# leggedrobotics/open3d_slam_private

Measured on AMD Instinct MI355X. Metric: ICP iterations/sec (scan-to-map), higher is better.
Workload: dtype f32

## Files before the change

open3d_slam_private_amd/capi.py:

```python
from __future__ import annotations

import ctypes as C
import math
import os
import subprocess

import numpy as np

_HERE = os.path.dirname(os.path.abspath(__file__))
_SO = os.environ.get("O3D_REG_LIB") or os.path.join(_HERE, "lib", "libo3dslam_reg.so")

STATUS_NAMES = {0: "OK", 1: "EMPTY_TARGET", 2: "EMPTY_SOURCE", 3: "NO_CORRESPONDENCES", 4: "BAD_TRANSFORM",
                5: "NOT_CONFIGURED", 6: "BAD_ARGUMENT", 7: "MISSING_FIELD", 8: "DEVICE_ERROR", 9: "UNSUPPORTED",
                10: "OUT_OF_BOUNDS"}
OUT_OF_BOUNDS = 10
COST_P2PL, COST_GICP = 0, 1
COST_O3D_P2PL, COST_O3D_P2P = 2, 3
SMOOTH_LEN_MAX = 15


class RegError(RuntimeError):
    def __init__(self, status, msg=""):
        self.status = status
        super().__init__(f"{STATUS_NAMES.get(status, status)}: {msg}")
# ... 1528 lines not shown
        raise RegError(st, "reg_host_o3d_update")
    return U.reshape(4, 4).T.copy(), rank.value


def host_tail_plan(n, cus=256, tile=0):
    lib = load_library()
    lib.reg_host_tail_plan.argtypes = [C.c_int64, C.c_int32, C.c_int32, C.POINTER(C.c_int32)]
    lib.reg_host_tail_plan.restype = None
    out = (C.c_int32 * 4)()
    lib.reg_host_tail_plan(int(n), int(cus), int(tile), out)
    return bool(out[0]), int(out[1]), int(out[2]), int(out[3])


def host_predict_band(limit, prev=math.inf, prev2=math.inf, last_count=0, last_lo=math.inf, last_hi=math.inf, debug_narrow=0):
    lib = load_library()
    lib.reg_host_predict_band.argtypes = [C.c_float, C.c_float, C.c_float, C.c_uint32, C.c_float, C.c_float, C.c_int32,
                                          C.POINTER(C.c_float), C.POINTER(C.c_float)]
    lib.reg_host_predict_band.restype = None
    out = (C.c_float * 2)()
    lib.reg_host_predict_band(float(limit), float(prev), float(prev2), int(last_count), float(last_lo), float(last_hi),
                              int(debug_narrow), out, None)
    return np.float32(out[0]), np.float32(out[1])


def host_band_constants():
    lib = load_library()
    lib.reg_host_predict_band.argtypes = [C.c_float, C.c_float, C.c_float, C.c_uint32, C.c_float, C.c_float, C.c_int32,
                                          C.POINTER(C.c_float), C.POINTER(C.c_float)]
    lib.reg_host_predict_band.restype = None
    c = (C.c_float * 8)()
    lib.reg_host_predict_band(math.inf, math.inf, math.inf, 0, math.inf, math.inf, 0, None, c)
    names = ("band_cap", "wide_rel", "floor", "ratio_max", "centre_gain", "geom_rel", "guard_frac", "forced_wide")
    return {k: float(np.float32(v)) for k, v in zip(names, c)}
```

open3d_slam_private_amd/csrc/host_loop.hpp:

```cpp
#pragma once


static reg_status check_ready(reg_handle* h, bool need_prepared) {
    if (!h) return REG_BAD_ARGUMENT;
    if (!h->device_ok) return REG_DEVICE_ERROR;
    if (h->m == 0) {
        h->err = "no reference set (reg_set_target)";
        return REG_NOT_CONFIGURED;
    }
    if (h->n == 0) {
        h->err = "no reading set (reg_set_source)";
        return REG_NOT_CONFIGURED;
    }
    if (need_prepared && !h->prepared) {
        h->err = "reg_prepare has not been called for this reading";
        return REG_NOT_CONFIGURED;
    }
    return REG_OK;
}

static reg_status prepare_rowmajor(reg_handle* h, const float* T_init_row, const float* c_override = nullptr,
                                   int64_t n_global = 0, const IterState* init_state = nullptr) {
    reg_status s = check_ready(h, false);
    if (s != REG_OK) return s;
// ... 278 lines not shown
    const float* B = m->T_prev;
    float R[9];
    for (int i = 0; i < 3; ++i)
        for (int j = 0; j < 3; ++j) R[3 * i + j] = A[4 * i + 0] * B[4 * j + 0] + A[4 * i + 1] * B[4 * j + 1] + A[4 * i + 2] * B[4 * j + 2];
    float t[3];
    for (int i = 0; i < 3; ++i) t[i] = A[4 * i + 3] - (R[3 * i + 0] * B[3] + R[3 * i + 1] * B[7] + R[3 * i + 2] * B[11]);
    *trans = std::sqrt(t[0] * t[0] + t[1] * t[1] + t[2] * t[2]);
    const float sx = 0.5f * (R[7] - R[5]), sy = 0.5f * (R[2] - R[6]), sz = 0.5f * (R[3] - R[1]);
    *rot = std::sqrt(sx * sx + sy * sy + sz * sz);
}

static reg_status enqueue_tail(reg_handle* h, const TailPlan& pl, int max_iters) {
    if (!h->i_tail_sync.p) h->tail_sync_dirty = true;
    HIPCHK(h, h->i_tail_sync.reserve(2 * (size_t)kTailSyncBytes));
    if (h->tail_sync_dirty) {
        HIPCHK(h, hipMemsetAsync(h->i_tail_sync.p, 0, 2 * (size_t)kTailSyncBytes, h->stream));
        h->tail_sync_dirty = false;
    }
    const int sync_slot = h->tail_sync_slot;
    h->tail_sync_slot ^= 1;
    h->tail_sync_last = sync_slot;
    unsigned* const sync_cur = h->i_tail_sync.as<unsigned>() + (size_t)sync_slot * (kTailSyncBytes / 4);
    unsigned* const sync_next = h->i_tail_sync.as<unsigned>() + (size_t)(sync_slot ^ 1) * (kTailSyncBytes / 4);
    HIPCHK(h, h->i_tail_rows.reserve((size_t)2 * pl.grid * kTailHistRow * 8));
    HIPCHK(h, h->i_tail_band.reserve((size_t)2 * kTailBandCap * kTailRec * 4));
    const FilterCfg f = make_filter_cfg(h, 0);
    TailCfg cfg;
    cfg.n = h->n;
    cfg.chunk8 = pl.chunk8;
    cfg.wpc = pl.wpc;
    cfg.tile = pl.tile;
    cfg.max_iters = std::max(1, std::min(max_iters, kTailMaxIters));
    cfg.slack = coherent_slack(h);
    cfg.seq = ++h->seq;
    cfg.timeout_ticks = (unsigned long long)(h->env.tail_timeout_s * 1e8);
    uint8_t* hint = h->dbg.match_variant == 2 ? nullptr : h->i_hint.as<uint8_t>();
    const bool gicp = h->prm.cost == REG_COST_GICP;
    const float4* s_attr = gicp ? (const float4*)h->s_cov.as<float4>() : (const float4*)(h->has_snrm ? h->s_nrm.as<float4>() : nullptr);
    const float4* t_attr = gicp ? (const float4*)h->t_cov.as<float4>() : (const float4*)h->t_nrm.as<float4>();
    auto go = [&](auto kernel) {
        launch_timed(h, 3, kernel, dim3(pl.grid), dim3(kTailThreads), kTailLdsBytes, (const float4*)h->s_xyz.as<float4>(), s_attr,
                     h->i_iter.as<IterState>(), h->grid, t_attr, f, h->i_pos.as<int>(), h->i_d2.as<float>(), h->i_w.as<float>(), hint,
                     h->i_cache.as<float4>(), sync_cur, h->i_tail_rows.as<double>(), h->i_tail_band.as<float>(), h->d_mirror, cfg,
                     sync_next);
    };
    if (gicp)
        go(k_tail<true>);
    else
        go(k_tail<false>);
    HIPCHK(h, hipGetLastError());
    h->have_match = true;
    return REG_OK;
}

static reg_status enqueue_iteration(reg_handle* h, bool want_w) {
    reg_status s = enqueue_match(h);
    if (s != REG_OK) return s;
    if (h->prm.cost == REG_COST_P2PL && h->prm.use_trimmed) enqueue_select(h);
    return enqueue_linearize(h, want_w);
}

static inline unsigned long long mirror_seq(const reg_handle* h) {
    return __atomic_load_n(&h->h_mirror->seq, __ATOMIC_ACQUIRE);
}

static reg_status wait_seq(reg_handle* h, unsigned long long seq) {
// ... 168 lines not shown
                  std::fabs(in.limit_last - in.limit_prev) <= settle_tol * in.limit_last;
    }
    if (settled && in.any && (p.p2pl || p.fixed <= 0) && (p.can_fuse || tail_now)) {
        if (in.step_trans > p.settle_trans || in.step_rot > p.settle_rot) settled = false;
    }
    if (!(p.can_fuse || tail_now) || in.generic_left > 0 || !settled) return {SteerChoice::kGeneric, 1};
    const int rest = in.limit - (in.completed + in.inflight);
    if (tail_now) return {SteerChoice::kTail, rest};
    return {SteerChoice::kFused, p.fixed > 0 && !p.no_burst ? rest : 1};
}

static reg_status wait_tail(reg_handle* h, unsigned long long tail_seq, Lookahead& la, bool* tail_off) {
    const HostMirror* mir = h->h_mirror;
    for (unsigned spins = 0;; ++spins) {
        const unsigned long long m = mirror_seq(h);
        if (m >= tail_seq) break;
        if (m + 1 == tail_seq) {
            const HostMirror::SeqRecord* rec = &mir->ring[(tail_seq - 1) % kSeqRing];
            if (__atomic_load_n(&rec->seq, __ATOMIC_ACQUIRE) == tail_seq - 1 && (rec->done || rec->stall)) break;
        }
        __builtin_ia32_pause();
        if ((spins & 0xfff) == 0xfff) {
            const hipError_t e = hipStreamQuery(h->stream);
            if (e == hipSuccess) break;
            if (e != hipErrorNotReady) {
                h->tail_sync_dirty = true;
                h->err = std::string("device fault while waiting for the tail kernel: ") + hipGetErrorString(e);
                return REG_DEVICE_ERROR;
            }
        }
    }
    const bool reported = mirror_seq(h) >= tail_seq;
    const unsigned* sync_last = h->i_tail_sync.as<unsigned>() + (size_t)h->tail_sync_last * (kTailSyncBytes / 4);
    unsigned words[4] = {0, 0, 0, 0};
    if (!reported || h->env.coh_stats || mir->status == REG_DEVICE_ERROR)
        (void)hipMemcpy(words, sync_last + kTailErrWord, sizeof(words), hipMemcpyDeviceToHost);
    if (words[0] != 0 || (reported && mir->status == REG_DEVICE_ERROR)) {
        h->tail_sync_dirty = true;
        h->err = "persistent tail kernel: a grid barrier timed out (workgroups not co-resident? another process "
                 "running a persistent kernel on this GPU?); set O3D_NO_TAIL=1 to use the three-launch iteration";
        return REG_DEVICE_ERROR;
    }
    if (!reported && !(mir->stall && std::max(mirror_seq(h), la.seq0) > la.acked)) la.acked = h->seq;
    if (h->env.coh_stats)
        fprintf(stderr, "[o3dreg] tail launch: %u iterations, %u point searches (%.2f %% of the point-iterations), stall cause %u, band records of its last iteration %d\n", words[2],
                words[1], words[2] ? 100.0 * words[1] / ((double)words[2] * (double)h->n) : 0.0, words[3], reported ? mir->pad_nband : -1);
    if (reported) h->last_tail_iters += mir->pad3;
    if (reported && mir->stall && h->prm.fixed_iters <= 0) *tail_off = true;
#if O3D_TAIL_STAMPS
    {
        unsigned long long st[24];
        (void)hipMemcpy(st, sync_last + kTailStampWord, sizeof(st), hipMemcpyDeviceToHost);
        const double it_n = std::max(1, reported ? mir->pad3 : 1);
        static const char* names[12] = {"check", "search", "epilogue", "bandrec+comps", "sum+publish+drain", "arrive+wait", "row sums",
                                        "band-stage", "band-scan", "band-rank", "band-add", "solve+update"};
        for (int wg = 0; wg < 2; ++wg) {
            fprintf(stderr, "[o3dreg] tail stamps (us per iteration, %s workgroup):", wg ? "last" : "first");
            for (int i = 0; i < 12; ++i) fprintf(stderr, " %s %.2f", names[i], st[12 * wg + i] * 0.01 / it_n);
            fprintf(stderr, "\n");
        }
    }
#endif
    return REG_OK;
}

static reg_status loop_time_end(reg_handle* h, bool event_timing, std::chrono::steady_clock::time_point t_begin, float* loop_ms) {
    if (event_timing) {
        HIPCHK(h, hipEventRecord(h->ev1, h->stream));
        HIPCHK(h, hipEventSynchronize(h->ev1));
        (void)hipEventElapsedTime(loop_ms, h->ev0, h->ev1);
    } else {
        *loop_ms = std::chrono::duration<float, std::milli>(std::chrono::steady_clock::now() - t_begin).count();
    }
    return REG_OK;
}

static void loop_end_diagnostics(reg_handle* h, reg_result* res) {
    const HostMirror* mir = h->h_mirror;
    if (h->env.hints) {
// ... 31 lines not shown
            }
        }
        for (hipEvent_t e : h->prof_ev) (void)hipEventDestroy(e);
        h->prof_ev.clear();
        h->prof_kind.clear();
        h->profiling = false;
    }
}

static reg_status register_pm(reg_handle* h, const float* Ti, float T_out[16], reg_result* res);

extern "C" {

void reg_host_tail_plan(int64_t n, int32_t cus, int32_t tile, int32_t plan[4]) {
    const TailPlan pl = tail_plan_for(n, cus, 0, tile);
    plan[0] = pl.ok ? 1 : 0;
    plan[1] = pl.grid;
    plan[2] = pl.wpc;
    plan[3] = pl.chunk8;
}

REG_API void reg_host_predict_band(float limit, float prev, float prev2, uint32_t last_count, float last_lo, float last_hi,
                                   int32_t debug_narrow, float band[2], float consts[8]) {
    const Band b = predict_band(limit, prev, prev2, last_count, last_lo, last_hi, debug_narrow);
    if (band) {
        band[0] = b.lo;
        band[1] = b.hi;
    }
    if (consts) {
        const float c[8] = {(float)kTailBandCap, kTailWideRel, kBandFloor, kBandRatioMax, kBandCentreGain, kBandGeomRel, kBandGuardFrac,
                            kBandForcedWide};
        for (int i = 0; i < 8; ++i) consts[i] = c[i];
    }
}

reg_status reg_prepare(reg_handle* h, const float T_init[16]) {
    if (!h || !T_init) return REG_BAD_ARGUMENT;
    float Tr[16];
    col_to_row(T_init, Tr);
    return prepare_rowmajor(h, Tr);
}

reg_status reg_linearize(reg_handle* h, const float T_iter[16], float H[36], float b[6], double* err,
                         int64_t* n_inliers) {
    reg_status s = check_ready(h, true);
    if (s != REG_OK) return s;
    if (!T_iter) return REG_BAD_ARGUMENT;
    if (h->prm.cost == REG_COST_O3D_P2P) {
        h->err = "reg_linearize: point-to-point (Umeyama) has no normal equations";
        return REG_UNSUPPORTED;
    }
    if (h->pm_on) {
        h->err = "reg_linearize: not available with a libpointmatcher chain (reg_set_pm_chain)";
        return REG_UNSUPPORTED;
    }
    float Tr[16];
    col_to_row(T_iter, Tr);
    if (!m4_is_finite(Tr)) return REG_BAD_TRANSFORM;
    HIPCHK(h, hipSetDevice(h->prm.device));
    s = iterate_once(h, Tr, true);
    if (s != REG_OK) return s;
    const double* sums = h->h_mirror->sums;
    if (H && b) sums_to_system(sums, h->prm.cost, H, b);
    if (err) *err = sums[27];
    if (n_inliers) *n_inliers = (int64_t)llround(sums[28]);
    if (sums[28] == 0.0) {
// ... 221 lines not shown
```

open3d_slam_private_amd/csrc/host_target.hpp:

```cpp
#pragma once



struct DevBuf {
    void* p = nullptr;
    size_t cap = 0;
    hipError_t reserve(size_t bytes) {
        if (bytes <= cap) return hipSuccess;
        if (p) (void)hipFree(p);
        p = nullptr;
        cap = 0;
        hipError_t e = hipMalloc(&p, bytes ? bytes : 16);
        if (e == hipSuccess) cap = bytes;
        return e;
    }
    void release() {
        if (p) (void)hipFree(p);
        p = nullptr;
        cap = 0;
    }
    template <class T>
    T* as() const {
        return (T*)p;
    }
};

struct EnvSwitches {
    bool trace = false;
    bool event_timing = false;
    bool halo_occ = true;
    bool no_dynprune = false;
    bool no_empty_bound = false;
    bool no_witness = false;
    bool no_burst = false;
    bool hints = false;
    bool stamps = false;
    bool coh_stats = false;
    bool tail_always = false;
    bool update_generic = false;
    bool no_tail = false;
    int tail_wpc = 0;
    double dist_timeout_s = 30.0;
    float tail_timeout_s = 2.f;
    int xcd_tile_first = 32;
    int xcd_tile_later = 16;
    float settle_trans = 0.02f;
    float settle_rot = 4e-3f;
    int tail_min_iters = 8;
    int tail_tile = 0;
    bool no_gicp_tail = false;
    int gicp_tail_after = 1;
    float tail_settle_tol = 1.2f;
    int lookahead = 2;
    float settle_tol = 0.05f;
    float halo_ratio = 1.25f;
    float halo_rho = 0.4f;
    float reach_bins = 7.25f;
    float bin_occupancy = 8.f;
    float level_ratio = 2.0f;
    void read() {
        trace = getenv("O3D_TRACE") != nullptr;
        event_timing = getenv("O3D_EVENT_TIMING") != nullptr;
        no_burst = getenv("O3D_NO_BURST") != nullptr;
        no_dynprune = getenv("O3D_NO_DYNPRUNE") != nullptr;
        no_empty_bound = getenv("O3D_NO_EMPTY_BOUND") != nullptr;
        no_witness = getenv("O3D_NO_WITNESS") != nullptr;
        halo_occ = getenv("O3D_NO_HALO_OCC") == nullptr;
        hints = getenv("O3D_HINTS") != nullptr;
        stamps = getenv("O3D_STAMPS") != nullptr;
        coh_stats = getenv("O3D_COH_STATS") != nullptr;
        tail_always = getenv("O3D_TAIL_ALWAYS") != nullptr;
        no_tail = getenv("O3D_NO_TAIL") != nullptr;
        if (const char* v = getenv("O3D_UPDATE_GENERIC")) update_generic = atoi(v) != 0;
        if (const char* v = getenv("O3D_TAIL_WPC")) tail_wpc = std::max(0, atoi(v));
        if (const char* v = getenv("O3D_DIST_TIMEOUT_S")) dist_timeout_s = std::max(0.5, atof(v));
        if (const char* v = getenv("O3D_TAIL_SETTLE")) tail_settle_tol = (float)atof(v);
        if (const char* v = getenv("O3D_NO_GICP_TAIL")) no_gicp_tail = atoi(v) != 0;
        if (const char* v = getenv("O3D_TAIL_TILE")) tail_tile = std::max(0, atoi(v));
        if (const char* v = getenv("O3D_TAIL_MIN_ITERS")) tail_min_iters = std::max(0, atoi(v));
        if (const char* v = getenv("O3D_SETTLE_TRANS")) settle_trans = (float)atof(v);
        if (const char* v = getenv("O3D_SETTLE_ROT")) settle_rot = (float)atof(v);
        if (const char* v = getenv("O3D_XCD_TILE_FIRST")) xcd_tile_first = std::max(0, atoi(v));
        if (const char* v = getenv("O3D_XCD_TILE_LATER")) xcd_tile_later = std::max(0, atoi(v));
        if (const char* v = getenv("O3D_GICP_TAIL_AFTER")) gicp_tail_after = atoi(v);
        if (const char* v = getenv("O3D_TAIL_TIMEOUT_S")) tail_timeout_s = std::min(30.f, std::max(0.01f, (float)atof(v)));
        if (const char* v = getenv("O3D_KAHEAD")) lookahead = std::max(1, atoi(v));
        if (const char* v = getenv("O3D_SETTLE")) settle_tol = (float)atof(v);
        if (const char* v = getenv("O3D_HALO_RATIO")) halo_ratio = std::min(4.0f, std::max(0.5f, (float)atof(v)));
        if (const char* v = getenv("O3D_HALO_RHO")) halo_rho = std::min(1.0f, std::max(0.05f, (float)atof(v)));
        if (const char* v = getenv("O3D_REACH_BINS")) reach_bins = std::max(1.0f, (float)atof(v));
        if (const char* v = getenv("O3D_BIN_OCC")) bin_occupancy = std::min(64.0f, std::max(1.0f, (float)atof(v)));
        if (const char* v = getenv("O3D_LEVEL_RATIO")) level_ratio = std::min(4.0f, std::max(1.2f, (float)atof(v)));
    }
};

struct DistCtx;

struct reg_handle {
    reg_params prm;
    reg_debug_params dbg;
    EnvSwitches env;
    std::string err;
    hipStream_t stream = nullptr;
    bool own_stream = false;
    bool device_ok = false;
// ... 1299 lines not shown
```

open3d_slam_private_amd/csrc/kernels_tail.hpp:

```cpp
#pragma once

#ifndef O3D_TAIL_ACQ
#define O3D_TAIL_ACQ 0
#endif
#ifndef O3D_TAIL_THREADS
#define O3D_TAIL_THREADS 512
#endif
constexpr int kTailThreads = O3D_TAIL_THREADS;
#ifndef O3D_TAIL_SLOTS
#define O3D_TAIL_SLOTS 1024
#endif
#ifndef O3D_TAIL_WGS_PER_CU
#define O3D_TAIL_WGS_PER_CU 1
#endif
constexpr int kTailSlots = O3D_TAIL_SLOTS;
constexpr int kTailWgsPerCu = O3D_TAIL_WGS_PER_CU;
constexpr int kTailPts = kTailSlots / kTailThreads;
constexpr int kTailRec = 12;
constexpr int kTailHistRow = 32;
constexpr int kTailCoarse = 256;
constexpr int kTailMaxIters = 64;
constexpr int kTailSyncWords = 256;
constexpr int kTailRing = 4;
constexpr int kTailBandCntWord = 128;
constexpr int kTailAccRows = 16;
constexpr int kTailAccDoubles = kTailRing * kTailAccRows * kSums;
constexpr int kTailSyncBytes = kTailSyncWords * 4 + kTailAccDoubles * 8;
constexpr int kTailArriveStride = 16;
constexpr int kTailErrWord = 192;
constexpr int kTailSearchedWord = 193;
constexpr int kTailItersWord = 194;
constexpr int kTailCauseWord = 195;
constexpr int kTailStampWord = 200;
constexpr int kTailGroups = kTailThreads / 8;
constexpr int kTailBins = 1024;
#ifndef O3D_TAIL_STAMPS
#define O3D_TAIL_STAMPS 0
#endif
#ifndef O3D_TAIL_G4
#define O3D_TAIL_G4 0
#endif
#if O3D_TAIL_STAMPS
#define TAIL_STAMP(i)                                                      \
    do {                                                                   \
        const unsigned long long now_ = __builtin_amdgcn_s_memrealtime();  \
        stamp_acc[i] += now_ - stamp_last;                                 \
        stamp_last = now_;                                                 \
    } while (0)
#else
#define TAIL_STAMP(i) do { } while (0)
#endif

struct TailCfg {
    int64_t n;
    int chunk8;
    int wpc;
    int tile;
    int max_iters;
    float slack;
    unsigned long long seq;
    unsigned long long timeout_ticks;
};

struct TailLds {
    static constexpr int kRows = 0;
    static constexpr int kUnion = kRows + 5 * kTailSlots * 16;
    static constexpr int kUnionSeg = (kTailThreads / 8) * kSegWords<8> * 4, kUnionSeg4 = O3D_TAIL_G4 ? (kTailThreads / 4) * kSegWords<4> * 4 : 0;
    static constexpr int kUnionMax = kUnionSeg > kUnionSeg4 ? (kUnionSeg > kTailBandCap * 8 ? kUnionSeg : kTailBandCap * 8)
                                                            : (kUnionSeg4 > kTailBandCap * 8 ? kUnionSeg4 : kTailBandCap * 8);
    static constexpr int kUnionBytes = (kUnionMax + 255) & ~255;
    static constexpr int kD2 = kUnion + kUnionBytes;
    static constexpr int kFail = kD2 + kTailSlots * 4;
    static constexpr int kWcls = kFail + kTailSlots * 2;
    static constexpr int kHint = kWcls + kTailSlots;
    static constexpr int kSh = kHint + kTailSlots;
    static constexpr int kTot = kSh + 16 * kSums * 8;
    static constexpr int kState = kTot + kSums * 8;
    static constexpr int kStateBytes = (int)((sizeof(IterState) + 15) & ~size_t(15));
    static constexpr int kMisc = kState + kStateBytes;
    static constexpr int kWtot = kMisc + 64;
    static constexpr int kOff = kWtot + 64;
    static constexpr int kX = kOff + 272 * 4;
    static constexpr int kWork = kX + 96;
    static constexpr int kMirror = kWork + kUpdWorkBytes;
    static constexpr int kMirrorBytes = (int)((sizeof(HostMirror) + 15) & ~size_t(15));
    static constexpr int kHist = kMirror + kMirrorBytes;
    static constexpr int kTotal = kHist + kTailBins * 4;
    static constexpr int kBk = kUnion;
};
static_assert(TailLds::kBk + kTailBandCap * 8 - TailLds::kUnion <= TailLds::kUnionBytes, "phase-C scratch exceeds the union");
static_assert(kTailGroups * kSegWords<8> * 4 <= TailLds::kUnionBytes, "segment lists exceed the union");
static_assert(TailLds::kTotal * kTailWgsPerCu <= 160 * 1024, "LDS budget of one CU");
constexpr int kTailLdsBytes = TailLds::kTotal;

__device__ __forceinline__ double tail_ld_f64(const double* p) {
    const unsigned long long v = __hip_atomic_load(reinterpret_cast<unsigned long long*>(const_cast<double*>(p)), __ATOMIC_RELAXED,
                                                   __HIP_MEMORY_SCOPE_AGENT);
    return __longlong_as_double((long long)v);
}
__device__ __forceinline__ void tail_st_f64(double* p, double x) {
    __hip_atomic_store(reinterpret_cast<unsigned long long*>(p), (unsigned long long)__double_as_longlong(x), __ATOMIC_RELAXED,
                       __HIP_MEMORY_SCOPE_AGENT);
}
__device__ __forceinline__ unsigned long long tail_ld_u64(const void* p) {
    return __hip_atomic_load(reinterpret_cast<unsigned long long*>(const_cast<void*>(p)), __ATOMIC_RELAXED, __HIP_MEMORY_SCOPE_AGENT);
}
__device__ __forceinline__ void tail_st_u64(void* p, unsigned long long x) {
    __hip_atomic_store(reinterpret_cast<unsigned long long*>(p), x, __ATOMIC_RELAXED, __HIP_MEMORY_SCOPE_AGENT);
}
__device__ __forceinline__ unsigned tail_ld_u32(const unsigned* p) {
    return __hip_atomic_load(const_cast<unsigned*>(p), __ATOMIC_RELAXED, __HIP_MEMORY_SCOPE_AGENT);
}

__device__ __noinline__ __attribute__((flatten)) void tail_solve_update(IterState* sit, const double* tot, const uint32_t* misc, float* s_x, UpdWork* work,
                                               bool trim, unsigned n_band_raw, unsigned n_band_all) {
    const int lane = (int)(threadIdx.x & 63);
    const float r_limit_last = sit->limit_last, r_limit_sel = __uint_as_float(misc[2]);
    const int r_dbg_narrow = sit->debug_narrow_band & 1;
    const int r_fixed = sit->fixed_iters, r_iters = sit->iterations;
    const int r_xnc = sit->xicp_nc;
    const double r_tot28 = tot[28];
    float r_T[16];
#pragma unroll
    for (int i = 0; i < 16; ++i) r_T[i] = sit->T[i];
    const int r = lane >> 3, c = lane & 7;
    double a = 0.0;
// ... 250 lines not shown
            sit->chk.max_iter_reached = true;
            sit->done = 1;
        }
    }
}

template <bool kGicp>
__global__ void __launch_bounds__(kTailThreads, (kTailThreads / 256) * kTailWgsPerCu)
k_tail(const float4* __restrict__ src, const float4* __restrict__ src_nrm ,
       IterState* __restrict__ it_g, Grid g, const float4* __restrict__ tgt_nrm ,
       FilterCfg f, int* __restrict__ pos_io, float* __restrict__ d2_out,
       float* __restrict__ w_out, uint8_t* __restrict__ hint_g, float4* __restrict__ cache, unsigned* __restrict__ sync,
       double* __restrict__ hist_g , float* __restrict__ band_g ,
       HostMirror* host, TailCfg cfg, unsigned* __restrict__ sync_next ) {
    extern __shared__ __attribute__((aligned(16))) char lds[];
    float4* const st_rows = reinterpret_cast<float4*>(lds + TailLds::kRows);
    uint32_t* const seg_lds = reinterpret_cast<uint32_t*>(lds + TailLds::kUnion);
    unsigned long long* const bk = reinterpret_cast<unsigned long long*>(lds + TailLds::kBk);
    float* const d2s = reinterpret_cast<float*>(lds + TailLds::kD2);
    uint16_t* const fail = reinterpret_cast<uint16_t*>(lds + TailLds::kFail);
    uint8_t* const wcls = reinterpret_cast<uint8_t*>(lds + TailLds::kWcls);
    uint8_t* const hnt = reinterpret_cast<uint8_t*>(lds + TailLds::kHint);
    double (*const sh)[kSums] = reinterpret_cast<double (*)[kSums]>(lds + TailLds::kSh);
    double* const tot = reinterpret_cast<double*>(lds + TailLds::kTot);
    uint32_t* const s_state = reinterpret_cast<uint32_t*>(lds + TailLds::kState);
    IterState* const sit = reinterpret_cast<IterState*>(s_state);
    uint32_t* const misc = reinterpret_cast<uint32_t*>(lds + TailLds::kMisc);
    uint32_t* const wtot = reinterpret_cast<uint32_t*>(lds + TailLds::kWtot);
    uint32_t* const off = reinterpret_cast<uint32_t*>(lds + TailLds::kOff);
    float* const s_x = reinterpret_cast<float*>(lds + TailLds::kX);
    UpdWork* const work = reinterpret_cast<UpdWork*>(lds + TailLds::kWork);
    uint32_t* const mir_w = reinterpret_cast<uint32_t*>(lds + TailLds::kMirror);
    uint32_t* const hist = reinterpret_cast<uint32_t*>(lds + TailLds::kHist);
    double* const acc_g = reinterpret_cast<double*>(sync + kTailSyncWords);
    constexpr int kStateWords = (int)(sizeof(IterState) / 4);
    constexpr int kWaves = kTailThreads / 64;
    static_assert(kStateWords <= kTailThreads && kTailThreads >= 256, "state staging / count scan by the first threads");

    const int t = threadIdx.x, lane = t & 63, wave = t >> 6;
    const int nwg = (int)gridDim.x;
    const int xcls = (int)(blockIdx.x & 7), wq = (int)(blockIdx.x >> 3);
    const int64_t n = cfg.n;
    int64_t q[kTailPts];
    bool valid[kTailPts];
    float4 s[kTailPts], sn[kTailPts];
    float4 sc1[kTailPts];
#pragma unroll
    for (int u = 0; u < kTailPts; ++u) {
        const int sl = t + u * kTailThreads;
        const int64_t oc = (int64_t)(sl >> 3) * cfg.wpc + wq;
        const int64_t r_in = oc * 8 + (sl & 7);
        if (cfg.tile > 0) {
            const int64_t tl = oc / cfg.tile, rr = oc - tl * cfg.tile;
            q[u] = ((tl * 8 + xcls) * cfg.tile + rr) * 8 + (sl & 7);
        } else {
            q[u] = (int64_t)xcls * cfg.chunk8 + r_in;
        }
        valid[u] = r_in < cfg.chunk8 && q[u] < n;
        if (!valid[u]) q[u] = 0;
    }
    if (t < kStateWords) s_state[t] = reinterpret_cast<const uint32_t*>(it_g)[t];
#pragma unroll
    for (int u = 0; u < kTailPts; ++u) {
        const int sl = t + u * kTailThreads;
        float4 r0 = cache[q[u]], r1 = cache[(size_t)n + q[u]];
        const float4 r2 = cache[2 * (size_t)n + q[u]], r3 = cache[3 * (size_t)n + q[u]];
// ... 112 lines not shown
    auto reserve_records = [&](unsigned set, const bool (&mine)[kTailPts], unsigned (&slot)[kTailPts]) {
        unsigned long long bal[kTailPts];
        unsigned nw = 0;
#pragma unroll
        for (int u = 0; u < kTailPts; ++u) {
            bal[u] = __ballot(mine[u]);
            nw += (unsigned)__popcll(bal[u]);
        }
        unsigned base = 0;
        if (nw != 0u) {
            if (lane == 0) base = atomicAdd(&sync[kTailBandCntWord + 16 * set], nw);
            base = (unsigned)__shfl((int)base, 0);
        }
        unsigned before = 0;
#pragma unroll
        for (int u = 0; u < kTailPts; ++u) {
            slot[u] = base + before + (unsigned)__popcll(bal[u] & ((1ull << lane) - 1ull));
            before += (unsigned)__popcll(bal[u]);
        }
    };
    auto store_record = [&](int buf, unsigned slotb, const float (&F)[7], float md2, float w) {
        if (slotb >= (unsigned)kTailBandCap) return;
        float* rec = band_g + ((size_t)buf * kTailBandCap + slotb) * kTailRec;
        const float kept = w != 0.f ? 1.f : 0.f;
        const float v[12] = {F[0], F[1], F[2], F[3], F[4], F[5], F[6], md2, kept, 0.f, w != 0.f ? md2 : 0.f, 0.f};
#pragma unroll
        for (int k = 0; k < 6; ++k)
            tail_st_u64(rec + 2 * k, ((unsigned long long)__float_as_uint(v[2 * k + 1]) << 32) | __float_as_uint(v[2 * k]));
    };

    for (;; ++k_local) {
        tv = t;
        asm volatile("" : "+v"(tv));
        Xf T;
#pragma unroll
        for (int k = 0; k < 12; ++k) T.m[k] = __int_as_float(__builtin_amdgcn_readfirstlane(__float_as_int(sit->T[k])));
        const float band_lo = sit->band_lo, band_hi = sit->band_hi;
        const bool trim = !kGicp && sit->use_trim && sit->trim_ratio != 1.0f;
        const bool wide = trim && band_hi < INFINITY && (band_hi - band_lo) > kTailWideRel * band_lo;
        const uint32_t u_lo = __float_as_uint(band_lo), u_hi = __float_as_uint(band_hi);
        const double f_scale = (wide ? (double)kTailCoarse : 1.0) / (double)(u_hi > u_lo ? u_hi - u_lo : 1u);
        auto coarse_bin = [&](float d2) -> uint32_t {
            return min((uint32_t)((double)(__float_as_uint(d2) - u_lo) * f_scale), (uint32_t)(kTailCoarse - 1));
        };
        float3 p[kTailPts];
#pragma unroll
        for (int u = 0; u < kTailPts; ++u) {
            const int sl = t + u * kTailThreads;
            p[u] = xf_point(T, s[u].x, s[u].y, s[u].z);
            const float4 c = st_rows[sl], tq = st_rows[kTailSlots + sl], nn = st_rows[2 * kTailSlots + sl],
                         ru = st_rows[3 * kTailSlots + sl];
            const int pprev = __float_as_int(tq.w);
            bool pass = false;
            const float attr_ok = kGicp ? st_rows[4 * kTailSlots + sl].w : nn.w;
            if (valid[u] && c.w > 0.f && pprev >= 0 && attr_ok == 1.f) {
                const float dx = p[u].x - tq.x, dy = p[u].y - tq.y, dz = p[u].z - tq.z;
                float a = dx * dx;
                float b2 = dy * dy;
                float d2 = a + b2;
                a = dz * dz;
                d2 = d2 + a;
                const float ex = p[u].x - c.x, ey = p[u].y - c.y, ez = p[u].z - c.z;
                const float delta = __builtin_amdgcn_sqrtf(ex * ex + ey * ey + ez * ez);
                const float lhs = (__builtin_amdgcn_sqrtf(d2) + delta) * 1.00001f + 1e-30f;
                const float rhs = __builtin_amdgcn_sqrtf(c.w) * 0.99999f;
                pass = d2 <= g.max_d2 && lhs < rhs;
                if (ru.w == 1.f) {
                    const float fx = p[u].x - ru.x, fy = p[u].y - ru.y, fz = p[u].z - ru.z;
                    float a2 = fx * fx;
                    float b3 = fy * fy;
                    float r2 = a2 + b3;
                    a2 = fz * fz;
                    r2 = r2 + a2;
                    pass = pass && d2 < r2;
                }
                if (pass) d2s[sl] = d2;
            }
            if (valid[u] && !pass) {
                const unsigned at = atomicAdd(&misc[0], 1u);
                fail[at] = (uint16_t)sl;
                st_rows[sl] = make_float4(p[u].x, p[u].y, p[u].z, -1.f);
            }
        }
        __syncthreads();
        TAIL_STAMP(0);
        const int nf = (int)misc[0];
        n_searched += (t == 0) ? (unsigned)nf : 0u;
        auto search_rounds = [&](auto gtag) {
            constexpr int G = decltype(gtag)::value;
            constexpr int kGroups = kTailThreads / G;
            const int sub = t & (G - 1), grp = t / G;
            for (int base = 0; base < nf; base += kGroups) {
                const int fi = base + grp;
                if (fi < nf) {
                    const int slot = (int)fail[fi];
                    const float4 a0 = st_rows[slot];
                    const float3 p2 = make_float3(a0.x, a0.y, a0.z);
                    const int hv = (int)hnt[slot];
                    int lvl;
                    float cov2;
                    const Best bb = nearest_group<G, O3D_COH_PRUNE != 0, true>(g, p2, sub, -1, &lvl, seg_lds + grp * kSegWords<G>,
                                                                               hv >= 2 ? hv - 2 : -1, &cov2, cfg.slack);
                    if (sub == 0) {
                        hnt[slot] = (uint8_t)(lvl + 1);
                        st_rows[slot] = make_float4(p2.x, p2.y, p2.z, bb.pos >= 0 ? fminf(bb.third, cov2) : -1.f);
                        st_rows[kTailSlots + slot].w = __int_as_float(bb.pos);
                        st_rows[3 * kTailSlots + slot].w = __int_as_float(bb.pos2);
                        d2s[slot] = bb.pos >= 0 ? bb.d2 : INFINITY;
                    }
                }
            }
        };
#if O3D_TAIL_G4
        if (nf > kTailThreads / 8)
            search_rounds(std::integral_constant<int, 4>());
        else
#endif
            search_rounds(std::integral_constant<int, 8>());
        __syncthreads();
#pragma unroll 1
        for (int fi = tv; fi < nf; fi += kTailThreads) {
            const int slot = (int)fail[fi];
            const int pos = __float_as_int(st_rows[kTailSlots + slot].w), pos2 = __float_as_int(st_rows[3 * kTailSlots + slot].w);
            const size_t pc = (size_t)(pos >= 0 ? pos : 0), pc2 = (size_t)(pos2 >= 0 ? pos2 : 0);
            const float4 t2 = g.pts[pc2];
            float4 tq = kGicp ? g.pts[pc] : tgt_nrm[2 * pc];
            float4 nn = kGicp ? tgt_nrm[2 * pc] : tgt_nrm[2 * pc + 1];
            if (kGicp) {
                float4 c1 = tgt_nrm[2 * pc + 1];
                c1.w = 1.f;
                st_rows[4 * kTailSlots + slot] = c1;
            } else {
                nn.w = 1.f;
            }
            tq.w = __int_as_float(pos);
            st_rows[kTailSlots + slot] = tq;
            st_rows[2 * kTailSlots + slot] = nn;
            st_rows[3 * kTailSlots + slot] = pos2 >= 0 ? make_float4(t2.x, t2.y, t2.z, 1.f)
                                                       : make_float4(INFINITY, INFINITY, INFINITY, 1.f);
        }
        __syncthreads();
        TAIL_STAMP(1);
        float rF[kTailPts][7], md2v[kTailPts], wv[kTailPts];
        int clsv[kTailPts];
        const unsigned set = epoch & (kTailRing - 1);
        int buf = (int)(epoch & 1u);
        {
            double v[kSums];
#pragma unroll
            for (int k = 0; k < kSums; ++k) v[k] = 0.0;
#pragma unroll
            for (int u = 0; u < kTailPts; ++u) {
                const int sl = t + u * kTailThreads;
#pragma unroll
                for (int k = 0; k < 7; ++k) rF[u][k] = 0.f;
                const float4 tq = st_rows[kTailSlots + sl], nn = st_rows[2 * kTailSlots + sl];
                const int mpos = valid[u] ? __float_as_int(tq.w) : -1;
                const float md2 = d2s[sl];
                float w = 0.f;
                int cls = 2;
                if (kGicp) {
                    if (valid[u] && mpos >= 0) {
                        w = 1.f;
                        cls = 0;
                        tail_gicp_factor(T, s[u], sn[u], sc1[u], tq, nn, st_rows[4 * kTailSlots + sl], md2, v);
                    }
                } else if (valid[u] && mpos >= 0) {
                    w = 1.f;
                    if (f.use_maxdist && !(md2 <= f.outlier_max_d2)) w = 0.f;
                    if (f.use_normal) {
                        const float3 nr = normalize3(xf_rot(T, sn[u].x, sn[u].y, sn[u].z));
                        const float3 nt = normalize3(make_float3(nn.x, nn.y, nn.z));
                        float a = nr.x * nt.x;
                        float bb2 = nr.y * nt.y;
                        float val = a + bb2;
                        a = nr.z * nt.z;
                        val = val + a;
                        if (val < f.cos_max_angle) w = 0.f;
                    }
                    cls = md2 < band_lo ? 0 : (md2 < band_hi ? 1 : 2);
                    if (w != 0.f && cls != 2) {
                        float a = p[u].y * nn.z, bq = p[u].z * nn.y;
                        rF[u][0] = a - bq;
                        a = p[u].z * nn.x; bq = p[u].x * nn.z;
                        rF[u][1] = a - bq;
                        a = p[u].x * nn.y; bq = p[u].y * nn.x;
                        rF[u][2] = a - bq;
                        rF[u][3] = nn.x; rF[u][4] = nn.y; rF[u][5] = nn.z;
                        const float dx = p[u].x - tq.x, dy = p[u].y - tq.y, dz = p[u].z - tq.z;
                        float r = dx * nn.x;
                        float t2 = dy * nn.y;
                        r = r + t2;
                        t2 = dz * nn.z;
                        r = r + t2;
                        rF[u][6] = r;
                    }
                    v[29] += 1.0;
                    if (cls == 0) v[31] += 1.0;
                    if (w != 0.f && cls == 0) accumulate(v, rF[u], md2);
                }
                if (!(valid[u] && mpos >= 0)) d2s[sl] = INFINITY;
                wcls[sl] = (uint8_t)((w != 0.f && cls != 2 ? 1 : 0) | (cls << 1));
                md2v[u] = md2;
                wv[u] = w;
                clsv[u] = cls;
                if (wide && cls == 1) atomicAdd(&hist[coarse_bin(md2)], 1u);
            }
            unsigned slot[kTailPts];
            if (!wide) {
                bool mine[kTailPts];
#pragma unroll
                for (int u = 0; u < kTailPts; ++u) mine[u] = clsv[u] == 1;
                reserve_records(set, mine, slot);
            }
            publish_sums(v);
            if (!wide) {
#pragma unroll
                for (int u = 0; u < kTailPts; ++u)
                    if (clsv[u] == 1) store_record(buf, slot[u], rF[u], md2v[u], wv[u]);
            }
        }
        TAIL_STAMP(2);
        if (wide) {
            __syncthreads();
            if (t < kTailCoarse / 8) {
                unsigned long long pk = 0ull;
#pragma unroll
                for (int j = 0; j < 8; ++j) {
                    const uint32_t c2 = hist[8 * t + j];
                    hist[8 * t + j] = 0u;
                    pk |= (unsigned long long)min(c2, 255u) << (8 * j);
                }
                tail_st_u64(hist_g + ((size_t)buf * nwg + blockIdx.x) * kTailHistRow + tv, pk);
            }
        }
        if (t == 0) {
            misc[0] = 0u;
            misc[5] = 0u;
            misc[9] = 0u;
            misc[2] = __float_as_uint(INFINITY);
        }
        TAIL_STAMP(3);
        if (!exchange(set)) {
            exit_reason = 4;
            if (t == 0) __hip_atomic_fetch_add(&sync[kTailErrWord], 1u, __ATOMIC_RELAXED, __HIP_MEMORY_SCOPE_AGENT);
            break;
        }
        TAIL_STAMP(5);
        uint32_t sel_bin = 0;
        bool stall = false;
        unsigned rset = set;
        unsigned long long rv[6] = {0ull, 0ull, 0ull, 0ull, 0ull, 0ull};
        unsigned n_band_raw = 0;
        auto load_records_spec = [&]() {
            n_band_raw = tail_ld_u32(&sync[kTailBandCntWord + 16 * rset]);
            const float* rec = band_g + ((size_t)buf * kTailBandCap + (unsigned)tv) * kTailRec;
#pragma unroll
            for (int k = 0; k < 6; ++k) rv[k] = tail_ld_u64(rec + 2 * k);
        };
        if (!wide) load_records_spec();
        reduce_sums(set, false);
        TAIL_STAMP(6);
        if (trim && wide && (uint32_t)llround(tot[29]) != 0u) {
            {
                const unsigned* wbase = reinterpret_cast<const unsigned*>(hist_g + (size_t)buf * nwg * kTailHistRow) + (tv & 63);
                constexpr int kG = kTailThreads / 64, kL = (256 * kTailWgsPerCu) / kG;
                unsigned c4[4] = {0, 0, 0, 0};
                bool sat = false;
                for (int u0 = 0; u0 < kL; u0 += 8) {
                    unsigned wv2[8];
// ... 174 lines not shown
                    const float d2r = __uint_as_float((unsigned)(r6[3] >> 32)), keptr = __uint_as_float((unsigned)r6[4]);
                    if (i < n_band && d2r <= limit && keptr != 0.f) {
                        const float F[7] = {__uint_as_float((unsigned)r6[0]), __uint_as_float((unsigned)(r6[0] >> 32)),
                                            __uint_as_float((unsigned)r6[1]), __uint_as_float((unsigned)(r6[1] >> 32)),
                                            __uint_as_float((unsigned)r6[2]), __uint_as_float((unsigned)(r6[2] >> 32)),
                                            __uint_as_float((unsigned)r6[3])};
                        accumulate(v, F, d2r);
                    }
                }
                wave_reduce32(v);
                if ((lane & 1) == 0) sh[wave][lane >> 1] = v[0];
                __syncthreads();
                if (t < kSums) {
                    double v2 = 0.0;
#pragma unroll
                    for (int w2 = 0; w2 < kWaves; ++w2) v2 += sh[w2][t];
                    tot[t] += v2;
                }
                __syncthreads();
            }
        }
        TAIL_STAMP(10);
        if (t < kSums) sit->sums[t] = tot[t];
        if (wave == 0) {
            if (kGicp)
                tail_solve_update_gicp(sit, tot, reinterpret_cast<double*>(s_x), work);
            else
                tail_solve_update(sit, tot, misc, s_x, work, trim, n_band_raw, wide ? misc[12] : n_band_raw);
        }
        __syncthreads();
        TAIL_STAMP(11);
        if (sit->done) {
            exit_reason = 1;
            ++k_local;
            break;
        }
        if (k_local + 1 >= cfg.max_iters) {
            exit_reason = 3;
            ++k_local;
            break;
        }
    }
    if (exit_reason == 2 || exit_reason == 4) {
        if (t == 0) {
            sit->stall = 1;
            sit->band_count = 0;
        }
        __syncthreads();
    }
#pragma unroll
    for (int u = 0; u < kTailPts; ++u) {
        if (!valid[u]) continue;
        const int sl = t + u * kTailThreads;
        const float4 tq = st_rows[kTailSlots + sl];
        const int cls = (int)(wcls[sl] >> 1);
        float w = (wcls[sl] & 1) ? 1.f : 0.f;
        if (cls == 1 && !(d2s[sl] <= __uint_as_float(misc[2]))) w = 0.f;
        pos_io[q[u]] = __float_as_int(tq.w);
        d2_out[q[u]] = d2s[sl];
        if (w_out) w_out[q[u]] = w;
        if (hint_g) hint_g[q[u]] = hnt[sl];
    }
    if (exit_reason == 3) {
        for (int sl = t; sl < kTailSlots; sl += kTailThreads) {
            const int64_t oc = (int64_t)(sl >> 3) * cfg.wpc + wq;
            const int64_t r_in = oc * 8 + (sl & 7);
            int64_t qq;
            if (cfg.tile > 0) {
                const int64_t tl = oc / cfg.tile, rr = oc - tl * cfg.tile;
                qq = ((tl * 8 + xcls) * cfg.tile + rr) * 8 + (sl & 7);
            } else {
                qq = (int64_t)xcls * cfg.chunk8 + r_in;
            }
            if (r_in < cfg.chunk8 && qq < n) {
#pragma unroll
                for (int r = 0; r < 4; ++r) cache[(size_t)r * (size_t)n + qq] = st_rows[r * kTailSlots + sl];
            }
        }
    }
    if (t == 0 && n_searched) atomicAdd(&sync[kTailSearchedWord], n_searched);
#if O3D_TAIL_STAMPS
    if (t == 0 && (blockIdx.x == 0 || blockIdx.x == gridDim.x - 1)) {
        unsigned long long* out = reinterpret_cast<unsigned long long*>(sync + kTailStampWord) + (blockIdx.x == 0 ? 0 : 12);
        for (int i = 0; i < 12; ++i) out[i] = stamp_acc[i];
    }
#endif
    if (blockIdx.x != 0) return;
    for (int w2 = t; w2 < kTailSyncBytes / 4; w2 += kTailThreads) sync_next[w2] = 0u;
    if (t == 0) sync[kTailItersWord] = (unsigned)k_local;
    if (wave != 0) return;
    if (lane == 0) {
        HostMirror* m = reinterpret_cast<HostMirror*>(mir_w);
        for (int i = 0; i < 16; ++i) m->T[i] = sit->T[i];
        for (int i = 0; i < 16; ++i) m->T_prev[i] = sit->T_prev[i];
        m->iterations = sit->iterations;
        m->done = sit->done;
        m->status = exit_reason == 4 ? (int)REG_DEVICE_ERROR : sit->status;
        m->rank_last = sit->rank_last;
        m->converged = sit->chk.converged ? 1 : 0;
        m->max_iter_reached = sit->chk.max_iter_reached ? 1 : 0;
        m->stall = sit->stall;
        m->band_count = (int)sit->band_count;
        m->limit_last = sit->limit_last;
        m->limit_prev = sit->limit_prev;
        m->band_lo = sit->band_lo;
        m->band_hi = sit->band_hi;
        m->pad_nband = (int)sit->band_count;
        m->pad2 = exit_reason;
        for (int i = 0; i < 6; ++i) {
            m->localizable[i] = sit->xicp_flags[i];
            m->xicp_comb[i] = sit->xicp_comb[i];
            m->xicp_high[i] = sit->xicp_high[i];
        }
// ... 30 lines not shown
```

Measured before the change: 19040.

## Skip nearest-neighbour searches for points certainly trimmed in the tail kernel

In the persistent tail kernel, a point whose cached match fails the coherence check is no longer re-searched if a distance bound shows it will certainly fall above the trim band's upper edge. Such points are marked trimmed (class 2) and counted. A final verification pass runs on convergence to re-check skipped points, using the final transform kept in LDS. This cuts k-d/grid search work per iteration, at the cost of extra LDS, a possible extra pass at convergence, and more branching. An environment variable turns it off.

After: 18760. 0.985x the previous value.

```diff
diff --git a/open3d_slam_private_amd/capi.py b/open3d_slam_private_amd/capi.py
--- a/open3d_slam_private_amd/capi.py
+++ b/open3d_slam_private_amd/capi.py
@@ -1584,3 +1584,18 @@
     lib.reg_host_predict_band(math.inf, math.inf, math.inf, 0, math.inf, math.inf, 0, None, c)
     names = ("band_cap", "wide_rel", "floor", "ratio_max", "centre_gain", "geom_rel", "guard_frac", "forced_wide")
     return {k: float(np.float32(v)) for k, v in zip(names, c)}
+
+
+def host_trim_skip(d_a, delta, band_hi, d2, max_d2, has_match):
+    lib = load_library()
+    fp, bp = C.POINTER(C.c_float), C.POINTER(C.c_uint8)
+    lib.reg_host_trim_skip.argtypes = [C.c_int64, fp, fp, fp, fp, C.c_float, bp, bp]
+    lib.reg_host_trim_skip.restype = None
+    arrs = np.broadcast_arrays(np.asarray(d_a, np.float32), np.asarray(delta, np.float32), np.asarray(band_hi, np.float32),
+                               np.asarray(d2, np.float32), np.asarray(has_match, np.uint8))
+    a, b, c, d = (np.ascontiguousarray(x, dtype=np.float32).ravel() for x in arrs[:4])
+    m = np.ascontiguousarray(arrs[4], dtype=np.uint8).ravel()
+    out = np.zeros(a.size, np.uint8)
+    lib.reg_host_trim_skip(a.size, a.ctypes.data_as(fp), b.ctypes.data_as(fp), c.ctypes.data_as(fp), d.ctypes.data_as(fp),
+                           float(max_d2), m.ctypes.data_as(bp), out.ctypes.data_as(bp))
+    return out.astype(bool).reshape(arrs[0].shape)
diff --git a/open3d_slam_private_amd/csrc/host_loop.hpp b/open3d_slam_private_amd/csrc/host_loop.hpp
--- a/open3d_slam_private_amd/csrc/host_loop.hpp
+++ b/open3d_slam_private_amd/csrc/host_loop.hpp
@@ -334,6 +334,7 @@
     cfg.tile = pl.tile;
     cfg.max_iters = std::max(1, std::min(max_iters, kTailMaxIters));
     cfg.slack = coherent_slack(h);
+    cfg.trim_skip = h->env.no_trim_skip ? 0 : 1;
     cfg.seq = ++h->seq;
     cfg.timeout_ticks = (unsigned long long)(h->env.tail_timeout_s * 1e8);
     uint8_t* hint = h->dbg.match_variant == 2 ? nullptr : h->i_hint.as<uint8_t>();
@@ -568,7 +569,7 @@
     }
     const bool reported = mirror_seq(h) >= tail_seq;
     const unsigned* sync_last = h->i_tail_sync.as<unsigned>() + (size_t)h->tail_sync_last * (kTailSyncBytes / 4);
-    unsigned words[4] = {0, 0, 0, 0};
+    unsigned words[5] = {0, 0, 0, 0, 0};
     if (!reported || h->env.coh_stats || mir->status == REG_DEVICE_ERROR)
         (void)hipMemcpy(words, sync_last + kTailErrWord, sizeof(words), hipMemcpyDeviceToHost);
     if (words[0] != 0 || (reported && mir->status == REG_DEVICE_ERROR)) {
@@ -579,8 +580,8 @@
     }
     if (!reported && !(mir->stall && std::max(mirror_seq(h), la.seq0) > la.acked)) la.acked = h->seq;
     if (h->env.coh_stats)
-        fprintf(stderr, "[o3dreg] tail launch: %u iterations, %u point searches (%.2f %% of the point-iterations), stall cause %u, band records of its last iteration %d\n", words[2],
-                words[1], words[2] ? 100.0 * words[1] / ((double)words[2] * (double)h->n) : 0.0, words[3], reported ? mir->pad_nband : -1);
+        fprintf(stderr, "[o3dreg] tail launch: %u iterations, %u point searches (%.2f %% of the point-iterations), %u skipped as certainly trimmed, stall cause %u, band records of its last iteration %d\n", words[2],
+                words[1], words[2] ? 100.0 * words[1] / ((double)words[2] * (double)h->n) : 0.0, words[4], words[3], reported ? mir->pad_nband : -1);
     if (reported) h->last_tail_iters += mir->pad3;
     if (reported && mir->stall && h->prm.fixed_iters <= 0) *tail_off = true;
 #if O3D_TAIL_STAMPS
@@ -678,6 +679,11 @@
                             kBandForcedWide};
         for (int i = 0; i < 8; ++i) consts[i] = c[i];
     }
+}
+
+REG_API void reg_host_trim_skip(int64_t n, const float* d_a, const float* delta, const float* band_hi, const float* d2, float max_d2,
+                                const uint8_t* has_match, uint8_t* out) {
+    for (int64_t i = 0; i < n; ++i) out[i] = trim_skip_certain(d_a[i], delta[i], band_hi[i], d2[i], max_d2, has_match[i] != 0) ? 1 : 0;
 }
 
 reg_status reg_prepare(reg_handle* h, const float T_init[16]) {
diff --git a/open3d_slam_private_amd/csrc/host_target.hpp b/open3d_slam_private_amd/csrc/host_target.hpp
--- a/open3d_slam_private_amd/csrc/host_target.hpp
+++ b/open3d_slam_private_amd/csrc/host_target.hpp
@@ -39,6 +39,7 @@
     bool tail_always = false;
     bool update_generic = false;
     bool no_tail = false;
+    bool no_trim_skip = false;
     int tail_wpc = 0;
     double dist_timeout_s = 30.0;
     float tail_timeout_s = 2.f;
@@ -71,6 +72,7 @@
         coh_stats = getenv("O3D_COH_STATS") != nullptr;
         tail_always = getenv("O3D_TAIL_ALWAYS") != nullptr;
         no_tail = getenv("O3D_NO_TAIL") != nullptr;
+        no_trim_skip = getenv("O3D_NO_TRIM_SKIP") != nullptr;
         if (const char* v = getenv("O3D_UPDATE_GENERIC")) update_generic = atoi(v) != 0;
         if (const char* v = getenv("O3D_TAIL_WPC")) tail_wpc = std::max(0, atoi(v));
         if (const char* v = getenv("O3D_DIST_TIMEOUT_S")) dist_timeout_s = std::max(0.5, atof(v));
diff --git a/open3d_slam_private_amd/csrc/kernels_tail.hpp b/open3d_slam_private_amd/csrc/kernels_tail.hpp
--- a/open3d_slam_private_amd/csrc/kernels_tail.hpp
+++ b/open3d_slam_private_amd/csrc/kernels_tail.hpp
@@ -31,6 +31,7 @@
 constexpr int kTailSearchedWord = 193;
 constexpr int kTailItersWord = 194;
 constexpr int kTailCauseWord = 195;
+constexpr int kTailSkippedWord = 196;
 constexpr int kTailStampWord = 200;
 constexpr int kTailGroups = kTailThreads / 8;
 constexpr int kTailBins = 1024;
@@ -58,6 +59,7 @@
     int tile;
     int max_iters;
     float slack;
+    int trim_skip;
     unsigned long long seq;
     unsigned long long timeout_ticks;
 };
@@ -85,13 +87,19 @@
     static constexpr int kMirror = kWork + kUpdWorkBytes;
     static constexpr int kMirrorBytes = (int)((sizeof(HostMirror) + 15) & ~size_t(15));
     static constexpr int kHist = kMirror + kMirrorBytes;
-    static constexpr int kTotal = kHist + kTailBins * 4;
+    static constexpr int kTfin = kHist + kTailBins * 4;
+    static constexpr int kTotal = kTfin + 64;
     static constexpr int kBk = kUnion;
 };
 static_assert(TailLds::kBk + kTailBandCap * 8 - TailLds::kUnion <= TailLds::kUnionBytes, "phase-C scratch exceeds the union");
 static_assert(kTailGroups * kSegWords<8> * 4 <= TailLds::kUnionBytes, "segment lists exceed the union");
 static_assert(TailLds::kTotal * kTailWgsPerCu <= 160 * 1024, "LDS budget of one CU");
 constexpr int kTailLdsBytes = TailLds::kTotal;
+
+__host__ __device__ inline bool trim_skip_certain(float d_a, float delta, float band_hi, float d2, float max_d2, bool has_match) {
+    if (!has_match || !(band_hi < INFINITY) || !(d2 <= max_d2)) return false;
+    return (d_a - delta) * 0.99999f > sqrtf(band_hi) * 1.00001f;
+}
 
 __device__ __forceinline__ double tail_ld_f64(const double* p) {
     const unsigned long long v = __hip_atomic_load(reinterpret_cast<unsigned long long*>(const_cast<double*>(p)), __ATOMIC_RELAXED,
@@ -408,6 +416,7 @@
     UpdWork* const work = reinterpret_cast<UpdWork*>(lds + TailLds::kWork);
     uint32_t* const mir_w = reinterpret_cast<uint32_t*>(lds + TailLds::kMirror);
     uint32_t* const hist = reinterpret_cast<uint32_t*>(lds + TailLds::kHist);
+    float* const t_fin = reinterpret_cast<float*>(lds + TailLds::kTfin);
     double* const acc_g = reinterpret_cast<double*>(sync + kTailSyncWords);
     constexpr int kStateWords = (int)(sizeof(IterState) / 4);
     constexpr int kWaves = kTailThreads / 64;
@@ -586,11 +595,15 @@
     for (;; ++k_local) {
         tv = t;
         asm volatile("" : "+v"(tv));
+        const bool fin = !kGicp && exit_reason == 1;
         Xf T;
 #pragma unroll
-        for (int k = 0; k < 12; ++k) T.m[k] = __int_as_float(__builtin_amdgcn_readfirstlane(__float_as_int(sit->T[k])));
+        for (int k = 0; k < 12; ++k) T.m[k] = __int_as_float(__builtin_amdgcn_readfirstlane(__float_as_int(fin ? t_fin[k] : sit->T[k])));
+        if (!kGicp && !fin && t < 12) t_fin[tv] = sit->T[tv];
         const float band_lo = sit->band_lo, band_hi = sit->band_hi;
         const bool trim = !kGicp && sit->use_trim && sit->trim_ratio != 1.0f;
+        const bool certify = !kGicp && trim && cfg.trim_skip != 0 && band_hi < INFINITY &&
+                             (sit->fixed_iters > 0 ? sit->iterations + 1 < sit->fixed_iters : sit->chk.count + 1 < sit->chk.max_iter);
         const bool wide = trim && band_hi < INFINITY && (band_hi - band_lo) > kTailWideRel * band_lo;
         const uint32_t u_lo = __float_as_uint(band_lo), u_hi = __float_as_uint(band_hi);
         const double f_scale = (wide ? (double)kTailCoarse : 1.0) / (double)(u_hi > u_lo ? u_hi - u_lo : 1u);
@@ -605,9 +618,11 @@
             const float4 c = st_rows[sl], tq = st_rows[kTailSlots + sl], nn = st_rows[2 * kTailSlots + sl],
                          ru = st_rows[3 * kTailSlots + sl];
             const int pprev = __float_as_int(tq.w);
-            bool pass = false;
+            bool pass = false, skip = false;
             const float attr_ok = kGicp ? st_rows[4 * kTailSlots + sl].w : nn.w;
-            if (valid[u] && c.w > 0.f && pprev >= 0 && attr_ok == 1.f) {
+            if (fin) {
+                pass = (wcls[sl] & 8) == 0;
+            } else if (valid[u] && c.w > 0.f && pprev >= 0 && attr_ok == 1.f) {
                 const float dx = p[u].x - tq.x, dy = p[u].y - tq.y, dz = p[u].z - tq.z;
                 float a = dx * dx;
                 float b2 = dy * dy;
@@ -628,9 +643,15 @@
                     r2 = r2 + a2;
                     pass = pass && d2 < r2;
                 }
-                if (pass) d2s[sl] = d2;
-            }
-            if (valid[u] && !pass) {
+                if (!kGicp && !pass && certify) {
+                    const float ax = c.x - tq.x, ay = c.y - tq.y, az = c.z - tq.z;
+                    skip = trim_skip_certain(__builtin_amdgcn_sqrtf(ax * ax + ay * ay + az * az), delta, band_hi, d2, g.max_d2, true);
+                }
+                if (pass || skip) d2s[sl] = d2;
+            }
+            if (!kGicp && !fin) wcls[sl] = skip ? (uint8_t)8 : (uint8_t)0;
+            if (skip) atomicAdd(&misc[13], 1u);
+            if (valid[u] && !pass && !skip) {
                 const unsigned at = atomicAdd(&misc[0], 1u);
                 fail[at] = (uint16_t)sl;
                 st_rows[sl] = make_float4(p[u].x, p[u].y, p[u].z, -1.f);
@@ -695,6 +716,7 @@
         }
         __syncthreads();
         TAIL_STAMP(1);
+        if (fin) break;
         float rF[kTailPts][7], md2v[kTailPts], wv[kTailPts];
         int clsv[kTailPts];
         const unsigned set = epoch & (kTailRing - 1);
@@ -733,6 +755,7 @@
                         if (val < f.cos_max_angle) w = 0.f;
                     }
                     cls = md2 < band_lo ? 0 : (md2 < band_hi ? 1 : 2);
+                    if (wcls[sl] & 8) cls = 2;
                     if (w != 0.f && cls != 2) {
                         float a = p[u].y * nn.z, bq = p[u].z * nn.y;
                         rF[u][0] = a - bq;
@@ -754,7 +777,7 @@
                     if (w != 0.f && cls == 0) accumulate(v, rF[u], md2);
                 }
                 if (!(valid[u] && mpos >= 0)) d2s[sl] = INFINITY;
-                wcls[sl] = (uint8_t)((w != 0.f && cls != 2 ? 1 : 0) | (cls << 1));
+                wcls[sl] = (uint8_t)((w != 0.f && cls != 2 ? 1 : 0) | (cls << 1) | (kGicp ? 0 : (wcls[sl] & 8)));
                 md2v[u] = md2;
                 wv[u] = w;
                 clsv[u] = cls;
@@ -790,6 +813,11 @@
         }
         if (t == 0) {
             misc[0] = 0u;
+            if (!kGicp) {
+                misc[14] += misc[13];
+                misc[15] = misc[13];
+                misc[13] = 0u;
+            }
             misc[5] = 0u;
             misc[9] = 0u;
             misc[2] = __float_as_uint(INFINITY);
@@ -1030,6 +1058,9 @@
         TAIL_STAMP(11);
         if (sit->done) {
             exit_reason = 1;
+            if (!kGicp && misc[15] != 0u) {
+                continue;
+            }
             ++k_local;
             break;
         }
@@ -1051,7 +1082,7 @@
         if (!valid[u]) continue;
         const int sl = t + u * kTailThreads;
         const float4 tq = st_rows[kTailSlots + sl];
-        const int cls = (int)(wcls[sl] >> 1);
+        const int cls = (int)(wcls[sl] >> 1) & 3;
         float w = (wcls[sl] & 1) ? 1.f : 0.f;
         if (cls == 1 && !(d2s[sl] <= __uint_as_float(misc[2]))) w = 0.f;
         pos_io[q[u]] = __float_as_int(tq.w);
@@ -1077,6 +1108,7 @@
         }
     }
     if (t == 0 && n_searched) atomicAdd(&sync[kTailSearchedWord], n_searched);
+    if (!kGicp && t == 0 && misc[14]) atomicAdd(&sync[kTailSkippedWord], misc[14]);
 #if O3D_TAIL_STAMPS
     if (t == 0 && (blockIdx.x == 0 || blockIdx.x == gridDim.x - 1)) {
         unsigned long long* out = reinterpret_cast<unsigned long long*>(sync + kTailStampWord) + (blockIdx.x == 0 ? 0 : 12);
```
